# yu45020/Text_Segmentation_Image_Inpainting

Measured on AMD Instinct MI355X. Metric: imgs/sec fwd+bwd on 512x512 partial-conv inpaint, higher is better.
Workload: dtype f32 (storage, accumulation, stencils, BatchNorm; matrix products = 6-term exact bf16 split on the bf16 MFMA, fp32-class error); 1 GPU; ImageFill 512x512 partial-conv inpainting train step (fwd+bwd, train-mode BN, L1 loss, grad all-reduce, fused SGD), 32 imgs/GPU, random line/ellipse hole masks; global_batch=32, parallelism=dp1, gemm_products=6, activation_storage=f32

## Files before the change

### include/tsii_hip.h

```cpp
#ifndef TSII_HIP_H
#define TSII_HIP_H

#include <stddef.h>
#include <stdint.h>

#ifdef __cplusplus
extern "C" {
#endif

#define TSII_ABI_VERSION 23

#define TSII_ACT_NONE 0
#define TSII_ACT_RELU 1
#define TSII_ACT_LEAKY 2
#define TSII_ACT_RELU6 3
#define TSII_ACT_SIGMOID 4

int tsii_version(void);
const char* tsii_last_error(void);

int tsii_set_gemm_products(int products);
int tsii_get_gemm_products(void);


int tsii_mask_channel_sum(const float* mask, int n, int h, int w, int c,
                          int64_t sn, int64_t sh, int64_t sw, int64_t sc,
                          float* plane, void* stream);

int tsii_mask_update(const float* p0, float a0, const float* p1, float a1,
                     int n, int h, int w,
                     int kh, int kw, int sh, int sw, int ph, int pw, int dh, int dw,
                     int ho, int wo, float post_scale, int fill_holes,
                     float* denom, float* new_mask, float* inv, void* stream);
// ... 55 lines not shown
                      int n, int h, int wd, int cout, float* y, void* ws, size_t ws_bytes, void* stream);
int tsii_head_cat_bwd_dx(const float* dy, const float* inv, const float* w, int c1, int c2, const float* r0, const float* r1,
                         int n, int h, int wd, int cout, float* dlow, float* dskip, void* ws, size_t ws_bytes, void* stream);
int tsii_head_cat_bwd_dw(const float* dy, const float* inv, const float* keep, const float* low, const float* skip,
                         int c1, int c2, const float* r0, const float* r1, int n, int h, int wd, int cout,
                         float* dwgt, float* dbias, void* ws, size_t ws_bytes, void* stream);
int tsii_head_cat_low_ok(int n, int h, int wd, int c1, int c2, int cout);
int tsii_head_cat_bwd_low_ok(int n, int h, int wd, int c1, int c2, int cout);
int tsii_head_cat_bwd_low(const float* dy, const float* inv, const float* keep, const float* low, const float* skip,
                          int c1, int c2, const float* r0_low, const float* r1, const float* w, int n, int h, int wd, int cout,
                          float* dwgt, float* dbias, float* dlow, void* ws, size_t ws_bytes, void* stream);
int tsii_head_cat_fwd_low_ok(int n, int h, int wd, int c1, int c2, int cout);
int tsii_head_cat_fwd_low(const float* low, const float* skip, int c1, int c2, const float* r0_low, const float* r1,
                          const float* w, const float* bias, const float* denom, const float* keep,
                          int n, int h, int wd, int cout, float* y, void* stream);
int tsii_head_cat_bwd_dw_low(const float* dy, const float* inv, const float* keep, const float* low, const float* skip,
                             int c1, int c2, const float* r0_low, const float* r1, int n, int h, int wd, int cout,
                             float* dwgt, float* dbias, void* ws, size_t ws_bytes, void* stream);

int tsii_stem_s2d(const float* x, const float* mfull, const float* r0, int split, const float* r1,
                  int n, int h, int w, int c, int pad, float* out, void* stream);
int tsii_stem_w_fwd(const float* w, int cout, int cin, int k, float* w2, void* stream);
int tsii_stem_w_bwd(const float* dw2, int cout, int cin, int k, float* dw, void* stream);

size_t tsii_bn_ws_bytes(int64_t m, int c);
int tsii_bn_stats(const float* y, int64_t m, int c, float* mean, float* var,
                  float* running_mean, float* running_var, float momentum,
                  void* ws, size_t ws_bytes, void* stream);
int tsii_bn_act_fwd(const float* y, int64_t m, int c, const float* mean, const float* var,
                    const float* gamma, const float* beta, float eps, int act, float slope,
                    const float* residual, float* out, void* stream);
int tsii_bn_act_bwd(const float* dout, const float* y, int64_t m, int c,
                    const float* mean, const float* var, const float* gamma, const float* beta,
                    float eps, int act, float slope, int training,
                    float* dy, float* dgamma, float* dbeta, void* ws, size_t ws_bytes, void* stream);

int64_t tsii_pw_stat_rows(int64_t m);
int tsii_pw_fwd_bn(const float* x, int64_t m, int k, const float* w, int n, const float* bias,
                   const float* r0, int split, const float* r1, const float* denom, const float* keep,
                   const float* in_scale, const float* in_shift, int in_act, float in_slope,
                   float* stat_part, float* y, void* ws, size_t ws_bytes, void* stream);
int tsii_pw_bwd_dw_bn(const float* dy, const float* x, int64_t m, int n, int k, const float* inv, const float* keep,
                      const float* r0, int split, const float* r1,
                      const float* in_scale, const float* in_shift, int in_act, float in_slope,
                      float* dw, float* dbias, void* ws, size_t ws_bytes, void* stream);
int64_t tsii_dw_stat_rows(int n, int ho, int wo, int c, int kh, int kw, int sh, int sw, int dh, int dw);
// ... 281 lines not shown
```

### text_segmentation_image_inpainting_amd/BaseModels.py

```python
from contextlib import contextmanager

from typing import NamedTuple, Optional

import torch
from torch import nn

from . import ops


class BaseModule(nn.Module):

    def __init__(self):
        super().__init__()
        self.act_fn = None

    def initialize_weights(self):
        for mod in self.modules():
            weight = getattr(mod, "weight", None)
            if weight is None or not weight.requires_grad:
                continue
            if isinstance(mod, nn.Conv2d):
                nn.init.kaiming_normal_(weight, mode="fan_out", nonlinearity="leaky_relu")
                if mod.bias is not None:
                    nn.init.zeros_(mod.bias)
# ... 249 lines not shown
    return to_nchw(h)


class DSConvBlock(BaseModule):

    def __init__(self, in_channels, out_channels, kernel_size, stride=1, padding=0,
                 dilation=1, bias=True, BN=False, activation_dep=None, activation_point=None):
        super().__init__()
        self.depth_wise_conv = nn.Sequential(
            *Conv_block(in_channels, in_channels, kernel_size, stride, padding,
                        dilation, in_channels, bias, BN=BN, activation=activation_dep))
        self.point_wise_conv = nn.Sequential(
            *Conv_block(in_channels, out_channels, kernel_size=1, stride=1, padding=0,
                        dilation=1, bias=bias, BN=BN, activation=activation_point))

    def forward(self, x):
        return run_chain(list(self.depth_wise_conv) + list(self.point_wise_conv), x)


def run_nhwc(layer, x, mp):
    if hasattr(layer, "forward_nhwc"):
        return layer.forward_nhwc(x, mp)
    if isinstance(layer, nn.Sequential):
        from .partial_convolution import PartialActivatedBN, PartialConv, PartialConv1x1, run_block
        if len(layer) == 2 and isinstance(layer[0], (PartialConv, PartialConv1x1)) and isinstance(layer[1], PartialActivatedBN):
            return run_block(layer, x, mp)
        for m in layer:
            x, mp = run_nhwc(m, x, mp)
        return x, mp
    raise NotImplementedError(f"{type(layer).__name__} is not part of the partial-convolution path")
```

### text_segmentation_image_inpainting_amd/_lib.py

```python
import ctypes
import os

import torch

_HERE = os.path.dirname(os.path.abspath(__file__))
LIB_PATH = os.environ.get("TSII_LIBRARY") or os.path.join(_HERE, "libtsii_hip.so")
ABI_VERSION = 23

_p, _i, _l, _f, _z = ctypes.c_void_p, ctypes.c_int, ctypes.c_int64, ctypes.c_float, ctypes.c_size_t
_GEOM = [_i] * 8

SIGNATURES = {
    "tsii_version": (_i, []),
    "tsii_last_error": (ctypes.c_char_p, []),
    "tsii_set_gemm_products": (_i, [_i]),
    "tsii_get_gemm_products": (_i, []),
    "tsii_mask_channel_sum": (_i, [_p, _i, _i, _i, _i, _l, _l, _l, _l, _p, _p]),
    "tsii_mask_update": (_i, [_p, _f, _p, _f, _i, _i, _i] + _GEOM + [_i, _i, _f, _i, _p, _p, _p, _p]),
    "tsii_plane_upsample2x": (_i, [_p, _i, _i, _i, _p, _p]),
    "tsii_mul_mask": (_i, [_p, _p, _l, _p, _p]),
    "tsii_pw_ws_bytes": (_z, [_i, _i]),
    "tsii_pw_fwd": (_i, [_p, _l, _i, _p, _i, _p, _p, _i, _p, _p, _p, _p, _p, _z, _p]),
    "tsii_pw_bwd_dx": (_i, [_p, _l, _i, _p, _i, _p, _p, _i, _p, _p, _p, _p]),
    "tsii_pw_bwd_dw_ws_bytes": (_z, [_l, _i, _i]),
    "tsii_pw_bwd_dw": (_i, [_p, _p, _l, _i, _i, _p, _p, _p, _i, _p, _p, _p, _p, _z, _p]),
    "tsii_pw_bwd_dxdw_ok": (_i, [_l, _i, _i, _l]),
    "tsii_pw_bwd_dxdw_tiles_per_block": (_i, [_l, _i, _i]),
    "tsii_pw_bwd_dxdw_ws_bytes": (_z, [_l, _i, _i]),
    "tsii_pw_bwd_dxdw": (_i, [_p, _p, _l, _i, _p, _i, _p, _p, _p, _i, _p, _p, _p, _p, _p, _z, _p]),
    "tsii_dw_fwd": (_i, [_p, _p, _p, _p, _p, _p, _i, _i, _i, _i] + _GEOM + [_i, _i, _p, _p, _p]),
    "tsii_dw_bwd_dx": (_i, [_p, _p, _p, _p, _i, _i, _i, _i] + _GEOM + [_i, _i, _p, _p, _p]),
    "tsii_dw_bwd_dw_ws_bytes": (_z, [_i, _i, _i, _i, _i, _i]),
    "tsii_dw_bwd_dw": (_i, [_p, _p, _p, _p, _p, _i, _i, _i, _i] + _GEOM + [_i, _i, _p, _p, _p, _z, _p]),
    "tsii_dense_ws_bytes": (_z, [_i, _i, _i, _i]),
    "tsii_dense_fwd": (_i, [_p, _p, _p, _i, _p, _p, _p, _p, _p, _i, _i, _i, _i, _i] + _GEOM + [_i, _i, _p, _p, _z, _p]),
    "tsii_dense_bwd_dx": (_i, [_p, _p, _p, _p, _p, _i, _p, _i, _i, _i, _i, _i] + _GEOM + [_i, _i, _p, _p, _z, _p]),
    "tsii_head_cat_ok": (_i, [_i, _i, _i, _i, _i, _i]),
    "tsii_head_cat_fwd": (_i, [_p, _p, _i, _i, _p, _p, _p, _p, _p, _p, _i, _i, _i, _i, _p, _p, _z, _p]),
    "tsii_head_cat_bwd_dx": (_i, [_p, _p, _p, _i, _i, _p, _p, _i, _i, _i, _i, _p, _p, _p, _z, _p]),
    "tsii_head_cat_bwd_dw": (_i, [_p, _p, _p, _p, _p, _i, _i, _p, _p, _i, _i, _i, _i, _p, _p, _p, _z, _p]),
    "tsii_head_cat_low_ok": (_i, [_i, _i, _i, _i, _i, _i]),
    "tsii_head_cat_fwd_low_ok": (_i, [_i, _i, _i, _i, _i, _i]),
    "tsii_head_cat_bwd_low_ok": (_i, [_i, _i, _i, _i, _i, _i]),
    "tsii_head_cat_bwd_low": (_i, [_p, _p, _p, _p, _p, _i, _i, _p, _p, _p, _i, _i, _i, _i, _p, _p, _p, _p, _z, _p]),
    "tsii_head_cat_fwd_low": (_i, [_p, _p, _i, _i, _p, _p, _p, _p, _p, _p, _i, _i, _i, _i, _p, _p]),
    "tsii_head_cat_bwd_dw_low": (_i, [_p, _p, _p, _p, _p, _i, _i, _p, _p, _i, _i, _i, _i, _p, _p, _p, _z, _p]),
    "tsii_dense_bwd_dw_ws_bytes": (_z, [_i, _i, _i, _i, _i, _i, _i]),
    "tsii_dense_bwd_dw": (_i, [_p, _p, _p, _p, _p, _p, _i, _p, _i, _i, _i, _i, _i] + _GEOM + [_i, _i, _p, _p, _p, _z, _p]),
    "tsii_stem_s2d": (_i, [_p, _p, _p, _i, _p, _i, _i, _i, _i, _i, _p, _p]),
    "tsii_stem_w_fwd": (_i, [_p, _i, _i, _i, _p, _p]),
    "tsii_stem_w_bwd": (_i, [_p, _i, _i, _i, _p, _p]),
    "tsii_bn_ws_bytes": (_z, [_l, _i]),
    "tsii_bn_stats": (_i, [_p, _l, _i, _p, _p, _p, _p, _f, _p, _z, _p]),
    "tsii_bn_act_fwd": (_i, [_p, _l, _i, _p, _p, _p, _p, _f, _i, _f, _p, _p, _p]),
    "tsii_bn_act_bwd": (_i, [_p, _p, _l, _i, _p, _p, _p, _p, _f, _i, _f, _i, _p, _p, _p, _p, _z, _p]),
    "tsii_pw_fwd_up": (_i, [_p, _l, _i, _p, _i, _p, _p, _i, _p, _p, _p, _p, _i, _i, _p, _p, _p, _z, _p]),
    "tsii_pool2x2_scaled": (_i, [_p, _p, _i, _i, _i, _i, _p, _p]),
    "tsii_pw_stat_rows": (_l, [_l]),
    "tsii_pw_fwd_bn": (_i, [_p, _l, _i, _p, _i, _p, _p, _i, _p, _p, _p, _p, _p, _i, _f, _p, _p, _p, _z, _p]),
    "tsii_pw_bwd_dw_bn": (_i, [_p, _p, _l, _i, _i, _p, _p, _p, _i, _p, _p, _p, _i, _f, _p, _p, _p, _z, _p]),
    "tsii_dw_stat_rows": (_l, [_i, _i, _i, _i, _i, _i, _i, _i, _i, _i]),
    "tsii_dw_bwd_stat_rows": (_l, [_i, _i, _i, _i, _i, _i, _i, _i, _i, _i, _i, _i]),
    "tsii_dw_fwd_bn": (_i, [_p, _p, _p, _p, _p, _p, _i, _i, _i, _i] + _GEOM + [_i, _i, _p, _p, _i, _f, _p, _p, _p, _p]),
    "tsii_dw_bwd_dw_bn": (_i, [_p, _p, _p, _p, _p, _i, _i, _i, _i] + _GEOM + [_i, _i, _p, _p, _i, _f, _p, _p, _p, _z, _p]),
    "tsii_dense_stat_rows": (_l, [_i, _i, _i, _i, _i, _i] + _GEOM + [_i, _i]),
    "tsii_dense_fwd_bn": (_i, [_p, _p, _p, _i, _p, _p, _p, _p, _p, _i, _i, _i, _i, _i] + _GEOM + [_i, _i, _p, _p, _p, _z, _p]),
    "tsii_bn_finalize_ws_bytes": (_z, [_l, _i]),
    "tsii_bn_finalize": (_i, [_p, _l, _i, _l, _p, _p, _p, _p, _f, _p, _p, _f, _p, _p, _p, _z, _p]),
    "tsii_dw_bwd_dx_bn": (_i, [_p, _p, _p, _p, _i, _i, _i, _i] + _GEOM + [_i, _i, _p, _p, _p, _p, _p, _f, _i, _f, _p, _p, _p, _p]),
    "tsii_dw_bwd_dxdw_ws_bytes": (_z, [_i, _i, _i, _i] + _GEOM),
    "tsii_dw_bwd_dxdw_bn": (_i, [_p, _p, _p, _p, _i, _i, _i, _i] + _GEOM + [_i, _i, _p, _p, _p, _p, _p, _f, _i, _f, _p, _p, _p, _p, _p, _z, _p]),
    "tsii_dw_bwd_dxdw_fold_ok": (_i, [_i, _i, _i, _i] + _GEOM),
    "tsii_dw_bwd_dxdw_bn2": (_i, [_p, _p, _p, _i, _f, _p, _p, _p, _i, _i, _i, _i] + _GEOM + [_i, _i, _p, _p, _p, _p, _p, _f, _i, _f, _p, _p, _p, _p, _p, _z, _p]),
    "tsii_bn_bwd_reduce_ws_bytes": (_z, [_l, _i]),
# ... 228 lines not shown
```

### text_segmentation_image_inpainting_amd/build_ext.py

```python
import hashlib
import json
import os
import re
import shutil
import subprocess
import sys
from concurrent.futures import ThreadPoolExecutor

HERE = os.path.dirname(os.path.abspath(__file__))
CSRC = os.path.join(HERE, "csrc")
OBJ = os.path.join(CSRC, "_obj")
LIB = os.path.join(HERE, "libtsii_hip.so")
ARCH = "gfx950"
FLAGS = ["-O3", "-std=c++17", "-fPIC", "--offload-arch=" + ARCH, "-Wall", "-Wno-unused-function"]
RESOURCE_REMARKS = ["-Rpass-analysis=kernel-resource-usage"]
NO_PACKED_F32 = ["-Xclang", "-target-feature", "-Xclang", "-packed-fp32-ops"]
MFMA_SOURCES = ("gemm.hip", "gemm_split.hip", "gemm_pc.hip", "head_mfma.hip", "bf16_gemm.hip", "gemm_dxdw.hip")


def flags_for(src):
    return FLAGS + (NO_PACKED_F32 if os.path.basename(src) in MFMA_SOURCES else [])


def _hipcc():
    for cand in (os.environ.get("HIPCC"), shutil.which("hipcc"), "/opt/rocm/bin/hipcc"):
        if cand and os.path.exists(cand):
            return cand
    raise RuntimeError("hipcc not found (need ROCm to build libtsii_hip.so)")


_REMARK = re.compile(r"remark: +([A-Za-z ]+?)(?: \[[^\]]*\])?: +(\S+)")
_REMARK_CONT = re.compile(r"^\s+\d+ \| |^\s+\| +\^")


def parse_resource_remarks(lines):
    keys = {"VGPRs": "vgprs", "AGPRs": "agprs", "ScratchSize": "scratch", "Occupancy": "occupancy", "LDS Size": "lds", "TotalSGPRs": "sgprs",
            "VGPRs Spill": "vgpr_spill", "SGPRs Spill": "sgpr_spill"}
    out, cur = {}, None
    for ln in lines:
        m = _REMARK.search(ln)
# ... 90 lines not shown
```

### text_segmentation_image_inpainting_amd/ops.py

```python
from typing import NamedTuple, Optional

import torch

from . import _lib
from ._lib import call, ptr

ACT_NONE, ACT_RELU, ACT_LEAKY, ACT_RELU6, ACT_SIGMOID = 0, 1, 2, 3, 4

FUSE_BN_BWD = True
FUSE_BN_BWD_PW = True
FUSE_DW_DXDW = True
FUSE_PW_DXDW = True
PW_DXDW_MIN_M = -1
FUSE_DW_BN2_FOLD = True
BF16_UNFUSE_K6C_ON_LARGE = False
FUSE_POOL_BN_BWD = True
USE_HEAD_MFMA = True
FUSE_HEAD_DLOW = True
USE_STEM_S2D = True


class Geom(NamedTuple):
    kh: int
    kw: int
    sh: int
    sw: int
    ph: int
    pw: int
    dh: int
    dw: int

    def out_hw(self, h, w):
        ho = (h + 2 * self.ph - self.dh * (self.kh - 1) - 1) // self.sh + 1
        wo = (w + 2 * self.pw - self.dw * (self.kw - 1) - 1) // self.sw + 1
        return ho, wo


def _pair(v):
    return (v, v) if isinstance(v, int) else tuple(v)


def make_geom(kernel_size, stride=1, padding=0, dilation=1) -> Geom:
# ... 512 lines not shown
        g = ctx.g
        gy = gy.contiguous()
        n, h, wd, cin = x.shape
        cout = w.shape[0]
        ho, wo = g.out_hw(h, wd)
        L, st = _lib.lib(), _lib.stream()
        dx = dw = db = None
        if ctx.needs_input_grad[0]:
            dx = torch.empty_like(x)
            nbytes = L.tsii_dense_ws_bytes(cin, cout, g.kh, g.kw)
            ws = _ws(nbytes, x)
            call("tsii_dense_bwd_dx", ptr(gy), ptr(inv), ptr(w), ptr(mfull), ptr(r0), ctx.split, ptr(r1),
                 n, h, wd, cin, cout, *g, ho, wo, ptr(dx), ptr(ws), nbytes, st)
        if ctx.needs_input_grad[1] or (ctx.has_bias and ctx.needs_input_grad[2]):
            dw = torch.empty_like(w)
            db = torch.empty(cout, dtype=torch.float32, device=x.device) if ctx.has_bias else None
            nbytes = L.tsii_dense_bwd_dw_ws_bytes(n, ho, wo, cin, cout, g.kh, g.kw)
            ws = _ws(nbytes, x)
            call("tsii_dense_bwd_dw", ptr(gy), ptr(inv), ptr(keep), ptr(x), ptr(mfull), ptr(r0), ctx.split, ptr(r1),
                 n, h, wd, cin, cout, *g, ho, wo, ptr(dw), ptr(db), ptr(ws), nbytes, st)
        return dx, dw, db, None, None, None, None, None, None, None, None, None


class _StemS2D(torch.autograd.Function):

    @staticmethod
    def forward(ctx, x, w, bias, mfull, r0, r1, denom, keep, inv, split, g, want_stats):
        _lib.check_device(x)
        x, w = x.contiguous(), w.contiguous()
        n, h, wd, cin = x.shape
        cout, k, pad = w.shape[0], g.kh, g.ph
        ka, c4 = (k + 1) // 2, 4 * cin
        h2, w2 = (h + 2 * pad) // 2, (wd + 2 * pad) // 2
        ho, wo = g.out_hw(h, wd)
        st, L = _lib.stream(), _lib.lib()
        x2 = torch.empty((n, h2, w2, c4), dtype=torch.float32, device=x.device)
        call("tsii_stem_s2d", ptr(x), ptr(mfull), ptr(r0), int(split), ptr(r1), n, h, wd, cin, pad, ptr(x2), st)
        wk = torch.empty((cout, c4, ka, ka), dtype=torch.float32, device=x.device)
        call("tsii_stem_w_fwd", ptr(w), cout, cin, k, ptr(wk), st)
        g2 = Geom(ka, ka, 1, 1, 0, 0, 1, 1)
        assert g2.out_hw(h2, w2) == (ho, wo)
        y = torch.empty((n, ho, wo, cout), dtype=torch.float32, device=x.device)
        nbytes = L.tsii_dense_ws_bytes(c4, cout, ka, ka)
        ws = _ws(nbytes, x)
        rows = int(L.tsii_dense_stat_rows(0, n, h2, w2, c4, cout, *g2, ho, wo)) if want_stats else 0
        part = None
        if rows > 0:
            part = torch.empty((rows, 4, cout), dtype=torch.float32, device=x.device)
            call("tsii_dense_fwd_bn", ptr(x2), None, None, 0, None, ptr(wk), ptr(bias), ptr(denom), ptr(keep),
                 n, h2, w2, c4, cout, *g2, ho, wo, ptr(part), ptr(y), ptr(ws), nbytes, st)
        else:
            call("tsii_dense_fwd", ptr(x2), None, None, 0, None, ptr(wk), ptr(bias), ptr(denom), ptr(keep),
                 n, h2, w2, c4, cout, *g2, ho, wo, ptr(y), ptr(ws), nbytes, st)
        ctx.save_for_backward(x2, inv, keep)
        ctx.cfg = (tuple(w.shape), g2, (n, h2, w2, c4, ho, wo), bias is not None)
        ctx.set_materialize_grads(False)
        if part is not None:
            ctx.mark_non_differentiable(part)
            return y, part
        return y

    @staticmethod
    def backward(ctx, gy, *_):
        if gy is None:
            return (None,) * 12
        x2, inv, keep = ctx.saved_tensors
        wshape, g2, (n, h2, w2, c4, ho, wo), has_bias = ctx.cfg
        cout, cin, k = wshape[0], wshape[1], wshape[2]
        gy = gy.contiguous()
        L, st = _lib.lib(), _lib.stream()
        dw = db = None
        if ctx.needs_input_grad[1] or (has_bias and ctx.needs_input_grad[2]):
            ka = g2.kh
            dwk = torch.empty((cout, c4, ka, ka), dtype=torch.float32, device=gy.device)
            db = torch.empty(cout, dtype=torch.float32, device=gy.device) if has_bias else None
            nbytes = L.tsii_dense_bwd_dw_ws_bytes(n, ho, wo, c4, cout, ka, ka)
            ws = _ws(nbytes, gy)
            call("tsii_dense_bwd_dw", ptr(gy), ptr(inv), ptr(keep), ptr(x2), None, None, 0, None,
                 n, h2, w2, c4, cout, *g2, ho, wo, ptr(dwk), ptr(db), ptr(ws), nbytes, st)
            dw = torch.empty(wshape, dtype=torch.float32, device=gy.device)
            call("tsii_stem_w_bwd", ptr(dwk), cout, cin, k, ptr(dw), st)
        return (None, dw, db) + (None,) * 9


class _DenseH(torch.autograd.Function):

    @staticmethod
    def forward(ctx, x, w, bias, g, want_stats):
        _lib.check_device(x, bf16_ok=True)
        x, w = x.contiguous(), w.contiguous()
        n, h, wd, cin = x.shape
        cout = w.shape[0]
        assert w.shape[1] == cin, "dense conv needs groups == 1"
        ho, wo = g.out_hw(h, wd)
        L = _lib.lib()
        y = torch.empty((n, ho, wo, cout), dtype=BF16, device=x.device)
        part = torch.empty((int(L.tsii_bf16_stat_rows(n * ho * wo)), 4, cout), dtype=torch.float32, device=x.device) if want_stats else None
        nbytes = L.tsii_bf16_dense_ws_bytes(cin, cout, g.kh, g.kw)
        ws = _ws(nbytes, x)
        call("tsii_bf16_dense_fwd", ptr(x), ptr(w), ptr(bias), n, h, wd, cin, cout, *g, ho, wo, ptr(part), ptr(y), ptr(ws), nbytes, _lib.stream())
        ctx.save_for_backward(x, w)
        ctx.g, ctx.has_bias = g, bias is not None
        ctx.set_materialize_grads(False)
        if want_stats:
# ... 140 lines not shown
    if cout % 8 != 0:
        if cout != 1 or want_stats:
            raise NotImplementedError(f"bf16 storage: {cout} output channels (multiples of 8, or a 1-channel head without BatchNorm)")
        w8 = torch.cat([w, w.new_zeros((7,) + tuple(w.shape[1:]))], 0)
        b8 = None if bias is None else torch.cat([bias, bias.new_zeros(7)], 0)
        return _ChannelToF32.apply(_DenseH.apply(x, w8, b8, g, False), 0)
    return _DenseH.apply(x, w, bias, g, want_stats)


def _stem_form(x, w, g: Geom):
    cin, cout = x.shape[-1], w.shape[0]
    return (USE_STEM_S2D and not x.requires_grad and g.kh == g.kw and g.kh % 2 == 1 and g.kh >= 3 and g.sh == g.sw == 2 and
            g.ph == g.pw == (g.kh - 1) // 2 and g.dh == g.dw == 1 and cin <= 4 and cout % 4 == 0 and cout >= 16 and
            (x.shape[1] + 2 * g.ph) % 2 == 0 and (x.shape[2] + 2 * g.pw) % 2 == 0)


def _bf16_stem_form(x, w, g: Geom):
    cin, cout = x.shape[-1], w.shape[0]
    return (not x.requires_grad and g.kh == g.kw and g.kh % 2 == 1 and g.kh >= 3 and g.sh == g.sw == 2 and
            g.ph == g.pw == (g.kh - 1) // 2 and g.dh == g.dw == 1 and cin <= 4 and cout % 8 == 0 and cout >= 16 and
            (x.shape[1] + 2 * g.ph) % 2 == 0 and (x.shape[2] + 2 * g.pw) % 2 == 0)


def pconv_dense(x, w, bias, mfull, r0, split, r1, denom, keep, inv, g: Geom, want_stats=False):
    data_layer = (_ACT_STORAGE == BF16 and x.dtype == torch.float32 and x.shape[-1] <= 4 and
                  mfull is None and r0 is None and denom is None)
    if data_layer and not _bf16_stem_form(x, w, g):
        raise NotImplementedError("bf16 activation storage: the data layer cannot enter it (needs an odd-k stride-2 'same' stem over "
                                  f"<= 4 channels with Cout % 8 == 0, even padded size and no input gradient; got k={g.kh}x{g.kw} "
                                  f"stride={g.sh} cin={x.shape[-1]} cout={w.shape[0]} requires_grad={x.requires_grad})")
    if _h(x) or data_layer:
        _no_masks("dense convolution", mfull, r0, r1, denom, keep)
        out = _dense_bf16(x, w, bias, g, want_stats)
        return (out, None) if (want_stats and not isinstance(out, tuple)) else out
    if _stem_form(x, w, g):
        out = _StemS2D.apply(x, w, bias, mfull, r0, r1, denom, keep, inv, split, g, want_stats)
    else:
        out = _Dense.apply(x, w, bias, mfull, r0, r1, denom, keep, inv, split, g, want_stats)
    if want_stats and not isinstance(out, tuple):
        return out, None
    return out


class _BNAct(torch.autograd.Function):
    @staticmethod
    def forward(ctx, y, gamma, beta, running_mean, running_var, residual, training, momentum, eps, act, slope, part=None):
        _lib.check_device(y)
        y = y.contiguous()
        c = y.shape[-1]
        m = y.numel() // c
        st = _lib.stream()
        if training:
            mean = torch.empty(c, dtype=torch.float32, device=y.device)
            var = torch.empty(c, dtype=torch.float32, device=y.device)
            if part is not None:
                rows = part.shape[0]
                nbytes = _lib.lib().tsii_bn_finalize_ws_bytes(rows, c)
# ... 803 lines not shown
```

### text_segmentation_image_inpainting_amd/partial_convolution.py

```python
import torch
from torch import nn

from . import ops
from .BaseModels import BaseModule, act_code, bn_state, to_nchw, to_nhwc
from .masks import MaskParts, as_parts

FUSE_BN = "1"
FUSE_UPCAT = True

inplace_batch_norm = False


def _public_forward(module, args, **kw):
    x, mask = args
    keep_parts = isinstance(mask, MaskParts)
    y, mp = module.forward_nhwc(to_nhwc(x), as_parts(mask), **kw)
    return to_nchw(y), (mp if keep_parts else mp.as_tensor())


class PartialConv(BaseModule):
    def __init__(self, in_channels, out_channels, kernel_size, stride=1,
                 padding=0, dilation=1, groups=1, bias=True, same_holes=False):
        super().__init__()
        self.feature_conv = nn.Conv2d(in_channels, out_channels, kernel_size, stride,
                                      padding, dilation, groups, bias)
        nn.init.kaiming_normal_(self.feature_conv.weight)
        self.same_holes = same_holes
        mask_in = 1 if same_holes else in_channels
        mask_out = 1 if same_holes else out_channels
        mask_groups = 1 if same_holes else groups
        self.mask_conv = nn.Conv2d(mask_in, mask_out, kernel_size, stride,
                                   padding, dilation, mask_groups, bias=False)
        torch.nn.init.constant_(self.mask_conv.weight, 1.0)
        for param in self.mask_conv.parameters():
            param.requires_grad = False

    fill_holes = True

    def _geom(self):
        fc = self.feature_conv
        return ops.make_geom(fc.kernel_size, fc.stride, fc.padding, fc.dilation)

    def forward_nhwc(self, x, mp, want_stats=False):
        fc = self.feature_conv
        w, b = fc.weight, fc.bias
        cin, cout, groups = fc.in_channels, fc.out_channels, fc.groups
        g = self._geom()
        if x.shape[-1] != cin or mp.channels != cin:
            raise RuntimeError(f"PartialConv expects {cin} input channels, got x:{x.shape[-1]} mask:{mp.channels}")
        if self.same_holes:
            p0, a0, p1, a1, post = mp.first_channel_plane(), 1.0, None, 0.0, float(cin)
        elif groups == 1:
            (p0, a0, p1, a1), post = mp.count_operands(), 1.0
        else:
            raise NotImplementedError("grouped PartialConv without same_holes (per-group mask counts, "
                                      "models/partial_convolution.py:63) is not used by any reference "
                                      "network and has no HIP kernel")
        denom, new_mask, inv = ops.mask_update(p0, a0, p1, a1, g, post, self.fill_holes)
        keep = new_mask if self.fill_holes else None
        pointwise = tuple(g) == (1, 1, 1, 1, 0, 0, 1, 1)
        part = None
        real = lambda t: t.materialize() if isinstance(t, ops.LazyBN) else t
        if isinstance(x, ops.VirtualCat):
            if (groups == 1 and mp.fusable and not want_stats and len(mp.parts) == 2 and mp.parts[0].channels == x.low.shape[3]
                    and ops.head_cat_ok(x, cout, g)):
                r0, _, r1 = mp.row_scale()
                y = ops.pconv_head_cat(x, w, b, r0, r1, denom, keep, inv)
                return y, MaskParts.from_plane(new_mask, cout)
            if (groups == 1 and pointwise and mp.fusable and len(mp.parts) == 2 and mp.parts[0].channels == x.low.shape[3]
                    and FUSE_UPCAT and ops.pointwise_up_ok(x, cout)):
                _, cl, r1 = mp.row_scale()
                z = ops.pconv_pointwise(x.low, w[:, :cl], None, x.low_plane, cl, None)
                y = ops.pconv_pointwise(x.skip, w[:, cl:], b, r1, cin - cl, None, denom, keep, inv, want_stats=want_stats, up_add=z)
                if want_stats:
                    y, part = y
                new_mp = MaskParts.from_plane(new_mask, cout)
                return (y, new_mp, part) if want_stats else (y, new_mp)
            x = x.materialize()
        if groups == 1:
            if mp.fusable:
                r0, split, r1 = mp.row_scale()
                if pointwise:
                    y = ops.pconv_pointwise(x, w, b, r0, split, r1, denom, keep, inv, want_stats=want_stats)
                    if want_stats:
                        y, part = y
                else:
                    y = ops.pconv_dense(real(x), w, b, None, r0, split, r1, denom, keep, inv, g, want_stats=want_stats)
                    if want_stats:
                        y, part = y
            else:
                mfull = mp.full_nhwc()
                if pointwise:
                    y = ops.pconv_pointwise(ops.mul_mask(real(x), mfull), w, b, None, 0, None, denom, keep, inv,
                                            want_stats=want_stats)
                    if want_stats:
                        y, part = y
                else:
                    y = ops.pconv_dense(real(x), w, b, mfull, None, 0, None, denom, keep, inv, g, want_stats=want_stats)
                    if want_stats:
                        y, part = y
        elif groups == cin == cout:
            if mp.fusable and len(mp.parts) == 1:
                y = ops.pconv_depthwise(x, w, b, mp.parts[0].plane, denom, keep, inv, g, want_stats=want_stats)
            else:
                y = ops.pconv_depthwise(ops.mul_mask(real(x), mp.full_nhwc()), w, b, None, denom, keep, inv, g,
                                        want_stats=want_stats)
            if want_stats:
                y, part = y
        else:
            raise NotImplementedError(f"PartialConv groups={groups} (neither 1 nor depth-wise) has no HIP kernel")
        new_mp = MaskParts.from_plane(new_mask, cout)
        return (y, new_mp, part) if want_stats else (y, new_mp)

    def forward(self, args):
        return _public_forward(self, args)


class PartialConv1x1(BaseModule):

    def __init__(self, in_channels, out_channels, kernel_size=1, stride=1,
                 padding=0, dilation=1, groups=1, bias=True):
# ... 71 lines not shown
        return ops.activation(x, act, slope), mp

    def forward(self, args):
        return _public_forward(self, args)


class DoubleUpSample(nn.Module):

    def __init__(self, scale_factor, mode="nearest"):
        super().__init__()
        if scale_factor != 2 or mode != "nearest":
            raise NotImplementedError("only the nearest x2 up-sampling the reference networks use has a HIP kernel")
        self.upsample = nn.Upsample(scale_factor=scale_factor, mode=mode)

    def forward_nhwc(self, x, mp):
        if not (mp.fusable and len(mp.parts) == 1 and mp.parts[0].planar):
            up = ops.upsample2x(mp.full_nhwc())
            from .masks import Part
            return ops.upsample2x(x), MaskParts([Part(mp.channels, full=up)])
        return ops.upsample2x(x), mp.upsample2x()

    def forward(self, args):
        return _public_forward(self, args)


def run_block(block, x, mp, allow_lazy=False, residual=None):
    mods = list(block)
    conv_types = (PartialConv, PartialConv1x1)
    if FUSE_BN != "0" and len(mods) == 2 and isinstance(mods[0], conv_types) and isinstance(mods[1], PartialActivatedBN):
        conv, bn = mods
        bn0 = bn.bn_act[0]
        if bn0.training or bn0.running_mean is None:
            y, m, part = conv.forward_nhwc(x, mp, want_stats=True)
        else:
            (y, m), part = conv.forward_nhwc(x, mp), None
        lazy, m = bn.forward_lazy(y, m, part)
        if allow_lazy and residual is None and FUSE_BN == "1" and ops.load_time_act(lazy.act, lazy.slope):
            return lazy, m
        return lazy.materialize(residual), m
    for mod in mods:
        if isinstance(x, ops.LazyBN) and not isinstance(mod, conv_types):
            x = x.materialize()
        x, mp = mod.forward_nhwc(x, mp)
    if isinstance(x, ops.LazyBN):
        x = x.materialize()
    if residual is not None:
# ... 19 lines not shown
```

Baseline: 573.8 imgs/s.

## Add fused stem backward kernel folding LeakyReLU grad into split-bf16 weight gradient

```diff
diff --git a/include/tsii_hip.h b/include/tsii_hip.h
--- a/include/tsii_hip.h
+++ b/include/tsii_hip.h
@@ -8,7 +8,7 @@
 extern "C" {
 #endif
 
-#define TSII_ABI_VERSION 23
+#define TSII_ABI_VERSION 24
 
 #define TSII_ACT_NONE 0
 #define TSII_ACT_RELU 1
@@ -110,6 +110,13 @@
                   int n, int h, int w, int c, int pad, float* out, void* stream);
 int tsii_stem_w_fwd(const float* w, int cout, int cin, int k, float* w2, void* stream);
 int tsii_stem_w_bwd(const float* dw2, int cout, int cin, int k, float* dw, void* stream);
+int tsii_stem_bwd_ok(const float* gy, const float* y, const float* x2, int n, int h2, int w2, int c4, int cout,
+                     int kh, int kw, int stride, int ho, int wo);
+int tsii_stem_bwd_tiles_per_block(int n, int ho, int wo);
+size_t tsii_stem_bwd_ws_bytes(int n, int ho, int wo);
+int tsii_stem_bwd(const float* gy, const float* y, float slope, const float* inv, const float* keep, const float* x2,
+                  int n, int h2, int w2, int c4, int cout, int kh, int kw, int stride, int ho, int wo,
+                  float* dwk, float* db, void* ws, size_t ws_bytes, void* stream);
 
 size_t tsii_bn_ws_bytes(int64_t m, int c);
 int tsii_bn_stats(const float* y, int64_t m, int c, float* mean, float* var,
diff --git a/text_segmentation_image_inpainting_amd/BaseModels.py b/text_segmentation_image_inpainting_amd/BaseModels.py
--- a/text_segmentation_image_inpainting_amd/BaseModels.py
+++ b/text_segmentation_image_inpainting_amd/BaseModels.py
@@ -295,9 +295,11 @@
     if hasattr(layer, "forward_nhwc"):
         return layer.forward_nhwc(x, mp)
     if isinstance(layer, nn.Sequential):
-        from .partial_convolution import PartialActivatedBN, PartialConv, PartialConv1x1, run_block
+        from .partial_convolution import PartialActivatedBN, PartialConv, PartialConv1x1, run_block, stem_act_block
         if len(layer) == 2 and isinstance(layer[0], (PartialConv, PartialConv1x1)) and isinstance(layer[1], PartialActivatedBN):
             return run_block(layer, x, mp)
+        if stem_act_block(layer, x):
+            return layer[0].forward_nhwc(x, mp, act_after=act_code(layer[1].act_fn))
         for m in layer:
             x, mp = run_nhwc(m, x, mp)
         return x, mp
diff --git a/text_segmentation_image_inpainting_amd/_lib.py b/text_segmentation_image_inpainting_amd/_lib.py
--- a/text_segmentation_image_inpainting_amd/_lib.py
+++ b/text_segmentation_image_inpainting_amd/_lib.py
@@ -5,7 +5,7 @@
 
 _HERE = os.path.dirname(os.path.abspath(__file__))
 LIB_PATH = os.environ.get("TSII_LIBRARY") or os.path.join(_HERE, "libtsii_hip.so")
-ABI_VERSION = 23
+ABI_VERSION = 24
 
 _p, _i, _l, _f, _z = ctypes.c_void_p, ctypes.c_int, ctypes.c_int64, ctypes.c_float, ctypes.c_size_t
 _GEOM = [_i] * 8
@@ -50,6 +50,10 @@
     "tsii_stem_s2d": (_i, [_p, _p, _p, _i, _p, _i, _i, _i, _i, _i, _p, _p]),
     "tsii_stem_w_fwd": (_i, [_p, _i, _i, _i, _p, _p]),
     "tsii_stem_w_bwd": (_i, [_p, _i, _i, _i, _p, _p]),
+    "tsii_stem_bwd_ok": (_i, [_p, _p, _p] + [_i] * 10),
+    "tsii_stem_bwd_tiles_per_block": (_i, [_i, _i, _i]),
+    "tsii_stem_bwd_ws_bytes": (_z, [_i, _i, _i]),
+    "tsii_stem_bwd": (_i, [_p, _p, _f, _p, _p, _p] + [_i] * 10 + [_p, _p, _p, _z, _p]),
     "tsii_bn_ws_bytes": (_z, [_l, _i]),
     "tsii_bn_stats": (_i, [_p, _l, _i, _p, _p, _p, _p, _f, _p, _z, _p]),
     "tsii_bn_act_fwd": (_i, [_p, _l, _i, _p, _p, _p, _p, _f, _i, _f, _p, _p, _p]),
diff --git a/text_segmentation_image_inpainting_amd/build_ext.py b/text_segmentation_image_inpainting_amd/build_ext.py
--- a/text_segmentation_image_inpainting_amd/build_ext.py
+++ b/text_segmentation_image_inpainting_amd/build_ext.py
@@ -15,7 +15,7 @@
 FLAGS = ["-O3", "-std=c++17", "-fPIC", "--offload-arch=" + ARCH, "-Wall", "-Wno-unused-function"]
 RESOURCE_REMARKS = ["-Rpass-analysis=kernel-resource-usage"]
 NO_PACKED_F32 = ["-Xclang", "-target-feature", "-Xclang", "-packed-fp32-ops"]
-MFMA_SOURCES = ("gemm.hip", "gemm_split.hip", "gemm_pc.hip", "head_mfma.hip", "bf16_gemm.hip", "gemm_dxdw.hip")
+MFMA_SOURCES = ("gemm.hip", "gemm_split.hip", "gemm_pc.hip", "head_mfma.hip", "bf16_gemm.hip", "gemm_dxdw.hip", "stem_bwd.hip")
 
 
 def flags_for(src):
diff --git a/text_segmentation_image_inpainting_amd/csrc/stem_bwd.hip b/text_segmentation_image_inpainting_amd/csrc/stem_bwd.hip
--- /dev/null
+++ b/text_segmentation_image_inpainting_amd/csrc/stem_bwd.hip
@@ -0,0 +1,286 @@
+#include "bf16_common.h"
+#include "gemm_tiles.h"
+#include "split_bf16.h"
+
+namespace tsii {
+
+static constexpr int SB_ROWS = 64;
+static constexpr int SB_SUB = 3 * SB_ROWS * 64;
+static constexpr int SB_C4 = 12, SB_KA = 4, SB_COUT = 64;
+static constexpr int SB_K = SB_C4 * SB_KA * SB_KA;
+static constexpr int SB_WIN_FLOATS = (SB_ROWS + SB_KA - 1) * SB_C4;
+static constexpr int SB_WIN_CHUNKS = (SB_WIN_FLOATS + 7) / 8;
+static constexpr int SB_WIN_ROW = SB_WIN_CHUNKS * 16;
+static constexpr int SB_WIN_PLANE = SB_KA * SB_WIN_ROW;
+static constexpr int SB_ROW_STEP = SB_C4 * 2;
+static constexpr int SB_SLAB = SB_K * SB_COUT + SB_COUT;
+
+#if defined(TSII_HIP_EMU)
+template <class... T> static inline void sb_lds_wait(T&...) {}
+#else
+__device__ __forceinline__ void sb_lds_wait(hu32x2& a, hu32x2& b, hu32x2& c, hu32x2& d, hu32x2& e, hu32x2& f) {
+    asm volatile("s_waitcnt lgkmcnt(0)" : "+v"(a), "+v"(b), "+v"(c), "+v"(d), "+v"(e), "+v"(f) : : "memory");
+}
+#endif
+
+__device__ __forceinline__ void sb_operand(hu32x2 (&lo)[3], hu32x2 (&hi)[3], bf16x8 (&o)[3]) {
+    sb_lds_wait(lo[0], hi[0], lo[1], hi[1], lo[2], hi[2]);
+#pragma unroll
+    for (int p = 0; p < 3; ++p) {
+        const u32x4 v = {lo[p][0], lo[p][1], hi[p][0], hi[p][1]};
+        o[p] = __builtin_bit_cast(bf16x8, v);
+    }
+}
+
+template <int KS>
+__device__ __forceinline__ void sb_step(const unsigned char* __restrict__ Gb, int tro0, int tro1, const unsigned char* (&Wa)[3], f32x16 (&acc)[3]) {
+    hu32x2 bl[3], bh[3];
+    bf16x8 b[3];
+    lds_read8_tr<KS * 1024>(bl[0], Gb + tro0);
+    lds_read8_tr<KS * 1024>(bh[0], Gb + tro1);
+    lds_read8_tr<KS * 1024 + SB_ROWS * 64>(bl[1], Gb + tro0);
+    lds_read8_tr<KS * 1024 + SB_ROWS * 64>(bh[1], Gb + tro1);
+    lds_read8_tr<KS * 1024 + 2 * SB_ROWS * 64>(bl[2], Gb + tro0);
+    lds_read8_tr<KS * 1024 + 2 * SB_ROWS * 64>(bh[2], Gb + tro1);
+    sb_operand(bl, bh, b);
+#pragma unroll
+    for (int s = 0; s < 3; ++s) {
+        constexpr int O = KS * 16 * SB_ROW_STEP;
+        hu32x2 al[3], ah[3];
+        bf16x8 a[3];
+        lds_read8_tr<O>(al[0], Wa[s]);
+        lds_read8_tr<O + 4 * SB_ROW_STEP>(ah[0], Wa[s]);
+        lds_read8_tr<O + SB_WIN_PLANE>(al[1], Wa[s]);
+        lds_read8_tr<O + SB_WIN_PLANE + 4 * SB_ROW_STEP>(ah[1], Wa[s]);
+        lds_read8_tr<O + 2 * SB_WIN_PLANE>(al[2], Wa[s]);
+        lds_read8_tr<O + 2 * SB_WIN_PLANE + 4 * SB_ROW_STEP>(ah[2], Wa[s]);
+        sb_operand(al, ah, a);
+#pragma unroll
+        for (int pq = 0; pq < 6; ++pq)
+            acc[s] = __builtin_amdgcn_mfma_f32_32x32x16_bf16(a[SplitTerm<6>::pa(pq)], b[SplitTerm<6>::pb(pq)], acc[s], 0, 0, 0);
+    }
+}
+
+__device__ __forceinline__ void sb_unpack(const float4 (&r)[2], float (&v)[8]) {
+    v[0] = r[0].x; v[1] = r[0].y; v[2] = r[0].z; v[3] = r[0].w; v[4] = r[1].x; v[5] = r[1].y; v[6] = r[1].z; v[7] = r[1].w;
+}
+
+template <bool ACT>
+__global__ __launch_bounds__(256, 2) void stem_bwd_kernel(const float* __restrict__ gy, const float* __restrict__ y, float slope,
+                                                          const float* __restrict__ inv, const float* __restrict__ keep,
+                                                          const float* __restrict__ x2, int ho, int wo, float* __restrict__ part,
+                                                          int ntiles, int tiles_per_block) {
+    __shared__ __attribute__((aligned(16))) unsigned char smem[2 * SB_SUB + 3 * SB_WIN_PLANE];
+    unsigned char* Gs = smem;
+    unsigned char* Wn = smem + 2 * SB_SUB;
+
+    const int tid = threadIdx.x, lane = tid & 63, wave = tid >> 6;
+    const int li = lane & 31, hi = lane >> 5;
+    const int wr = wave >> 1, wu = wave & 1;
+    const int tile_beg = (int)blockIdx.x * tiles_per_block;
+    const int tile_end = tile_beg + tiles_per_block < ntiles ? tile_beg + tiles_per_block : ntiles;
+    const int h2 = ho + SB_KA - 1, w2 = wo + SB_KA - 1, tiles_per_row = wo >> 6;
+
+    f32x16 acc[3];
+#pragma unroll
+    for (int s = 0; s < 3; ++s)
+#pragma unroll
+        for (int r = 0; r < 16; ++r) acc[s][r] = 0.f;
+    float dbacc[2][8];
+#pragma unroll
+    for (int h = 0; h < 2; ++h)
+#pragma unroll
+        for (int e = 0; e < 8; ++e) dbacc[h][e] = 0.f;
+
+    unsigned woff[2][2];
+    int wlds[2];
+    bool wvalid[2];
+#pragma unroll
+    for (int i = 0; i < 2; ++i) {
+        const int f = tid + 256 * i;
+        wvalid[i] = f < SB_KA * SB_WIN_CHUNKS;
+        const int fc = wvalid[i] ? f : SB_KA * SB_WIN_CHUNKS - 1;
+        const int ay = fc / SB_WIN_CHUNKS, ch = fc - ay * SB_WIN_CHUNKS;
+        woff[i][0] = (unsigned)((ay * w2 * SB_C4 + 8 * ch) * 4);
+        woff[i][1] = woff[i][0] + (8 * ch + 4 < SB_WIN_FLOATS ? 16u : 0u);
+        wlds[i] = ay * SB_WIN_ROW + ch * 16;
+    }
+
+    float4 rg[2][1][2], ry[2][1][2], rw[2][2];
+    float finv = 1.f, fkeep = 1.f;
+    auto prefetch = [&](int tile) {
+        const int64_t row0 = (int64_t)tile * SB_ROWS;
+        const int orow = tile / tiles_per_row, ox0 = (tile - orow * tiles_per_row) * SB_ROWS;
+        const int img = orow / ho, oy = orow - img * ho;
+        const char* xb = reinterpret_cast<const char*>(x2 + (((int64_t)img * h2 + oy) * w2 + ox0) * SB_C4);
+#pragma unroll
+        for (int i = 0; i < 2; ++i) {
+            rw[i][0] = *reinterpret_cast<const float4*>(xb + woff[i][0]);
+            rw[i][1] = *reinterpret_cast<const float4*>(xb + woff[i][1]);
+        }
+#pragma unroll
+        for (int h = 0; h < 2; ++h) {
+            split_load<SB_ROWS>(gy + row0 * SB_COUT, SB_COUT, 0, SB_ROWS, 32 * h, SB_COUT, rg[h]);
+            if constexpr (ACT) split_load<SB_ROWS>(y + row0 * SB_COUT, SB_COUT, 0, SB_ROWS, 32 * h, SB_COUT, ry[h]);
+        }
+        const int64_t row = row0 + (tid >> 2);
+        finv = inv != nullptr ? inv[row] : 1.f;
+        fkeep = keep != nullptr ? keep[row] : 1.f;
+    };
+
+    const int q = lane & 15, g1 = (lane >> 4) & 1;
+    int tro[2];
+#pragma unroll
+    for (int j = 0; j < 2; ++j) {
+        const int row = 8 * hi + (q >> 2) + 4 * j, chunk = 2 * g1 + ((q & 3) >> 1);
+        tro[j] = row * 64 + ((chunk ^ ((2 * hi + j) & 3)) << 4) + (q & 1) * 8;
+    }
+    const unsigned char* Gb = Gs + wu * SB_SUB;
+    const unsigned char* Wa[3];
+#pragma unroll
+    for (int s = 0; s < 3; ++s) {
+        const int b = 2 * (2 * s + wr) + g1, ay = b / 3, jb = b - 3 * ay;
+        Wa[s] = Wn + ay * SB_WIN_ROW + (8 * hi + (q >> 2)) * SB_ROW_STEP + (16 * jb + 4 * (q & 3)) * 2;
+    }
+
+    if (tile_beg < tile_end) prefetch(tile_beg);
+    for (int tile = tile_beg; tile < tile_end; ++tile) {
+        __syncthreads();
+#pragma unroll
+        for (int i = 0; i < 2; ++i) {
+            if (wvalid[i]) {
+                float v[8];
+                sb_unpack(rw[i], v);
+                u32x4 pl[3];
+                split8<3>(v, pl);
+#pragma unroll
+                for (int p = 0; p < 3; ++p) *reinterpret_cast<u32x4*>(Wn + p * SB_WIN_PLANE + wlds[i]) = pl[p];
+            }
+        }
+#pragma unroll
+        for (int h = 0; h < 2; ++h) {
+            float v[8];
+            sb_unpack(rg[h][0], v);
+            if constexpr (ACT) {
+                float a[8];
+                sb_unpack(ry[h][0], a);
+#pragma unroll
+                for (int e = 0; e < 8; ++e) v[e] = v[e] * (a[e] > 0.f ? 1.f : slope);
+                rg[h][0][0] = make_float4(v[0], v[1], v[2], v[3]);
+                rg[h][0][1] = make_float4(v[4], v[5], v[6], v[7]);
+            }
+#pragma unroll
+            for (int e = 0; e < 8; ++e) dbacc[h][e] += v[e] * fkeep;
+            const float s0[1] = {finv}, s1[1] = {finv};
+            const float4 z = make_float4(0.f, 0.f, 0.f, 0.f);
+            const float4 none[2] = {z, z};
+            split_store<SB_ROWS, 3, true, false>(Gs + h * SB_SUB, rg[h], 32 * h, 0x7fffffff, s0, s1, none, none, 1.f, 0.f, SB_ROWS, SB_COUT);
+        }
+        __syncthreads();
+        prefetch(tile + 1 < tile_end ? tile + 1 : tile);
+        __builtin_amdgcn_s_setprio(2);
+        sb_step<0>(Gb, tro[0], tro[1], Wa, acc);
+        sb_step<1>(Gb, tro[0], tro[1], Wa, acc);
+        sb_step<2>(Gb, tro[0], tro[1], Wa, acc);
+        sb_step<3>(Gb, tro[0], tro[1], Wa, acc);
+        __builtin_amdgcn_s_setprio(0);
+    }
+
+    float* pz = part + (int64_t)blockIdx.x * SB_SLAB;
+#pragma unroll
+    for (int s = 0; s < 3; ++s)
+#pragma unroll
+        for (int r = 0; r < 16; ++r) {
+            const int k = 32 * (2 * s + wr) + (r & 3) + 8 * (r >> 2) + 4 * hi;
+            pz[k * SB_COUT + 32 * wu + li] = acc[s][r];
+        }
+    __syncthreads();
+    float* Ds = reinterpret_cast<float*>(Gs);
+#pragma unroll
+    for (int h = 0; h < 2; ++h)
+#pragma unroll
+        for (int e = 0; e < 8; ++e) Ds[(tid >> 2) * SB_COUT + 32 * h + 8 * (tid & 3) + e] = dbacc[h][e];
+    __syncthreads();
+    if (tid < SB_COUT) {
+        float t = 0.f;
+        for (int r = 0; r < SB_ROWS; ++r) t += Ds[r * SB_COUT + tid];
+        pz[SB_K * SB_COUT + tid] = t;
+    }
+}
+
+__global__ void stem_bwd_finish_kernel(const float* __restrict__ red, float* __restrict__ dwk, float* __restrict__ db) {
+    const int o = (int)(blockIdx.x * blockDim.x + threadIdx.x);
+    if (o < SB_K * SB_COUT) {
+        const int co = o / SB_K, rem = o - co * SB_K;
+        const int c = rem >> 4, ay = (rem >> 2) & 3, ax = rem & 3;
+        dwk[o] = red[(48 * ay + 12 * ax + c) * SB_COUT + co];
+    } else if (o < SB_SLAB && db != nullptr) {
+        db[o - SB_K * SB_COUT] = red[o];
+    }
+}
+
+static bool sb_geom_ok(int n, int h2, int w2, int c4, int cout, int kh, int kw, int stride, int ho, int wo) {
+    if (n <= 0 || ho <= 0 || wo <= 0 || c4 != SB_C4 || cout != SB_COUT || kh != SB_KA || kw != SB_KA || stride != 1) return false;
+    if (wo % SB_ROWS != 0 || wo > (1 << 20) || h2 != ho + SB_KA - 1 || w2 != wo + SB_KA - 1) return false;
+    return (int64_t)n * ho * (wo / SB_ROWS) < (1ll << 31);
+}
+
+static void sb_plan(int n, int ho, int wo, int* nblocks, int* tiles_per_block) {
+    const int64_t ntiles = (int64_t)n * ho * (wo / SB_ROWS);
+    int64_t want = (int64_t)device_cus() * 2;
+    if (want > ntiles) want = ntiles;
+    const int64_t tpb = cdiv64(ntiles, want);
+    *tiles_per_block = (int)tpb;
+    *nblocks = (int)cdiv64(ntiles, tpb);
+}
+
+}
+
+using namespace tsii;
+
+extern "C" int tsii_stem_bwd_ok(const float* gy, const float* y, const float* x2, int n, int h2, int w2, int c4, int cout,
+                                int kh, int kw, int stride, int ho, int wo) {
+    if (gemm_products() != 6) return 0;
+    if (!sb_geom_ok(n, h2, w2, c4, cout, kh, kw, stride, ho, wo)) return 0;
+    return (gy != nullptr && x2 != nullptr && aligned16(gy) && aligned16(x2) && aligned16(y)) ? 1 : 0;
+}
+
+extern "C" int tsii_stem_bwd_tiles_per_block(int n, int ho, int wo) {
+    if (!sb_geom_ok(n, ho + SB_KA - 1, wo + SB_KA - 1, SB_C4, SB_COUT, SB_KA, SB_KA, 1, ho, wo)) return 0;
+    int nb = 0, tpb = 0;
+    sb_plan(n, ho, wo, &nb, &tpb);
+    return tpb;
+}
+
+extern "C" size_t tsii_stem_bwd_ws_bytes(int n, int ho, int wo) {
+    if (!sb_geom_ok(n, ho + SB_KA - 1, wo + SB_KA - 1, SB_C4, SB_COUT, SB_KA, SB_KA, 1, ho, wo)) return 0;
+    int nb = 0, tpb = 0;
+    sb_plan(n, ho, wo, &nb, &tpb);
+    return ((size_t)nb + 1) * SB_SLAB * sizeof(float);
+}
+
+extern "C" int tsii_stem_bwd(const float* gy, const float* y, float slope, const float* inv, const float* keep, const float* x2,
+                             int n, int h2, int w2, int c4, int cout, int kh, int kw, int stride, int ho, int wo,
+                             float* dwk, float* db, void* ws, size_t ws_bytes, void* stream) {
+    TSII_REQUIRE(gy && x2 && dwk && ws, "stem_bwd: null pointer");
+    TSII_REQUIRE(gemm_products() == 6, "stem_bwd: the 6-product split-bf16 arithmetic only (tsii_set_gemm_products)");
+    TSII_REQUIRE(sb_geom_ok(n, h2, w2, c4, cout, kh, kw, stride, ho, wo),
+                 "stem_bwd: n=%d x2 %dx%dx%d cout=%d taps %dx%d stride %d out %dx%d is not eligible (tsii_stem_bwd_ok)", n, h2, w2, c4, cout, kh,
+                 kw, stride, ho, wo);
+    TSII_REQUIRE(aligned16(gy) && aligned16(y) && aligned16(x2) && aligned16(ws), "stem_bwd: 16-byte aligned operands are required");
+    TSII_REQUIRE(ws_bytes >= tsii_stem_bwd_ws_bytes(n, ho, wo), "stem_bwd: workspace too small");
+    hipStream_t st = (hipStream_t)stream;
+    int nb = 0, tpb = 0;
+    sb_plan(n, ho, wo, &nb, &tpb);
+    const int ntiles = (int)((int64_t)n * ho * (wo / SB_ROWS));
+    float* part = (float*)ws;
+    float* red = part + (size_t)nb * SB_SLAB;
+    if (y != nullptr) hipLaunchKernelGGL((stem_bwd_kernel<true>), dim3(nb), dim3(256), 0, st, gy, y, slope, inv, keep, x2, ho, wo, part, ntiles, tpb);
+    else hipLaunchKernelGGL((stem_bwd_kernel<false>), dim3(nb), dim3(256), 0, st, gy, y, slope, inv, keep, x2, ho, wo, part, ntiles, tpb);
+    int rc = check_launch("stem_bwd");
+    if (rc) return rc;
+    rc = launch_reduce_rows(part, nb, SB_SLAB, red, st);
+    if (rc) return rc;
+    hipLaunchKernelGGL(stem_bwd_finish_kernel, dim3(cdiv(SB_SLAB, 256)), dim3(256), 0, st, red, dwk, db);
+    return check_launch("stem_bwd_finish");
+}
diff --git a/text_segmentation_image_inpainting_amd/ops.py b/text_segmentation_image_inpainting_amd/ops.py
--- a/text_segmentation_image_inpainting_amd/ops.py
+++ b/text_segmentation_image_inpainting_amd/ops.py
@@ -18,6 +18,7 @@
 USE_HEAD_MFMA = True
 FUSE_HEAD_DLOW = True
 USE_STEM_S2D = True
+FUSE_STEM_BWD = True
 
 
 class Geom(NamedTuple):
@@ -576,38 +577,72 @@
         return dx, dw, db, None, None, None, None, None, None, None, None, None
 
 
+def _stem_forward(ctx, x, w, bias, mfull, r0, r1, denom, keep, inv, split, g, want_stats):
+    _lib.check_device(x)
+    x, w = x.contiguous(), w.contiguous()
+    n, h, wd, cin = x.shape
+    cout, k, pad = w.shape[0], g.kh, g.ph
+    ka, c4 = (k + 1) // 2, 4 * cin
+    h2, w2 = (h + 2 * pad) // 2, (wd + 2 * pad) // 2
+    ho, wo = g.out_hw(h, wd)
+    st, L = _lib.stream(), _lib.lib()
+    x2 = torch.empty((n, h2, w2, c4), dtype=torch.float32, device=x.device)
+    call("tsii_stem_s2d", ptr(x), ptr(mfull), ptr(r0), int(split), ptr(r1), n, h, wd, cin, pad, ptr(x2), st)
+    wk = torch.empty((cout, c4, ka, ka), dtype=torch.float32, device=x.device)
+    call("tsii_stem_w_fwd", ptr(w), cout, cin, k, ptr(wk), st)
+    g2 = Geom(ka, ka, 1, 1, 0, 0, 1, 1)
+    assert g2.out_hw(h2, w2) == (ho, wo)
+    y = torch.empty((n, ho, wo, cout), dtype=torch.float32, device=x.device)
+    nbytes = L.tsii_dense_ws_bytes(c4, cout, ka, ka)
+    ws = _ws(nbytes, x)
+    rows = int(L.tsii_dense_stat_rows(0, n, h2, w2, c4, cout, *g2, ho, wo)) if want_stats else 0
+    part = None
+    if rows > 0:
+        part = torch.empty((rows, 4, cout), dtype=torch.float32, device=x.device)
+        call("tsii_dense_fwd_bn", ptr(x2), None, None, 0, None, ptr(wk), ptr(bias), ptr(denom), ptr(keep),
+             n, h2, w2, c4, cout, *g2, ho, wo, ptr(part), ptr(y), ptr(ws), nbytes, st)
+    else:
+        call("tsii_dense_fwd", ptr(x2), None, None, 0, None, ptr(wk), ptr(bias), ptr(denom), ptr(keep),
+             n, h2, w2, c4, cout, *g2, ho, wo, ptr(y), ptr(ws), nbytes, st)
+    ctx.cfg = (tuple(w.shape), g2, (n, h2, w2, c4, ho, wo), bias is not None)
+    return y, part, x2
+
+
+def _stem_backward(ctx, x2, inv, keep, gy, y=None, slope=0.0):
+    wshape, g2, (n, h2, w2, c4, ho, wo), has_bias = ctx.cfg
+    cout, cin, k = wshape[0], wshape[1], wshape[2]
+    if not (ctx.needs_input_grad[1] or (has_bias and ctx.needs_input_grad[2])):
+        return None, None
+    gy = gy.contiguous()
+    L, st = _lib.lib(), _lib.stream()
+    ka = g2.kh
+    dwk = torch.empty((cout, c4, ka, ka), dtype=torch.float32, device=gy.device)
+    db = torch.empty(cout, dtype=torch.float32, device=gy.device) if has_bias else None
+    if FUSE_STEM_BWD and L.tsii_stem_bwd_ok(ptr(gy), ptr(y), ptr(x2), n, h2, w2, c4, cout, ka, ka, 1, ho, wo):
+        nbytes = L.tsii_stem_bwd_ws_bytes(n, ho, wo)
+        ws = _ws(nbytes, gy)
+        call("tsii_stem_bwd", ptr(gy), ptr(y), float(slope), ptr(inv), ptr(keep), ptr(x2), n, h2, w2, c4, cout, ka, ka, 1, ho, wo,
+             ptr(dwk), ptr(db), ptr(ws), nbytes, st)
+    else:
+        if y is not None:
+            dy = torch.empty_like(gy)
+            call("tsii_act_bwd", ptr(gy), ptr(y), gy.numel(), ACT_LEAKY, float(slope), ptr(dy), st)
+            gy = dy
+        nbytes = L.tsii_dense_bwd_dw_ws_bytes(n, ho, wo, c4, cout, ka, ka)
+        ws = _ws(nbytes, gy)
+        call("tsii_dense_bwd_dw", ptr(gy), ptr(inv), ptr(keep), ptr(x2), None, None, 0, None,
+             n, h2, w2, c4, cout, *g2, ho, wo, ptr(dwk), ptr(db), ptr(ws), nbytes, st)
+    dw = torch.empty(wshape, dtype=torch.float32, device=gy.device)
+    call("tsii_stem_w_bwd", ptr(dwk), cout, cin, k, ptr(dw), st)
+    return dw, db
+
+
 class _StemS2D(torch.autograd.Function):
 
     @staticmethod
     def forward(ctx, x, w, bias, mfull, r0, r1, denom, keep, inv, split, g, want_stats):
-        _lib.check_device(x)
-        x, w = x.contiguous(), w.contiguous()
-        n, h, wd, cin = x.shape
-        cout, k, pad = w.shape[0], g.kh, g.ph
-        ka, c4 = (k + 1) // 2, 4 * cin
-        h2, w2 = (h + 2 * pad) // 2, (wd + 2 * pad) // 2
-        ho, wo = g.out_hw(h, wd)
-        st, L = _lib.stream(), _lib.lib()
-        x2 = torch.empty((n, h2, w2, c4), dtype=torch.float32, device=x.device)
-        call("tsii_stem_s2d", ptr(x), ptr(mfull), ptr(r0), int(split), ptr(r1), n, h, wd, cin, pad, ptr(x2), st)
-        wk = torch.empty((cout, c4, ka, ka), dtype=torch.float32, device=x.device)
-        call("tsii_stem_w_fwd", ptr(w), cout, cin, k, ptr(wk), st)
-        g2 = Geom(ka, ka, 1, 1, 0, 0, 1, 1)
-        assert g2.out_hw(h2, w2) == (ho, wo)
-        y = torch.empty((n, ho, wo, cout), dtype=torch.float32, device=x.device)
-        nbytes = L.tsii_dense_ws_bytes(c4, cout, ka, ka)
-        ws = _ws(nbytes, x)
-        rows = int(L.tsii_dense_stat_rows(0, n, h2, w2, c4, cout, *g2, ho, wo)) if want_stats else 0
-        part = None
-        if rows > 0:
-            part = torch.empty((rows, 4, cout), dtype=torch.float32, device=x.device)
-            call("tsii_dense_fwd_bn", ptr(x2), None, None, 0, None, ptr(wk), ptr(bias), ptr(denom), ptr(keep),
-                 n, h2, w2, c4, cout, *g2, ho, wo, ptr(part), ptr(y), ptr(ws), nbytes, st)
-        else:
-            call("tsii_dense_fwd", ptr(x2), None, None, 0, None, ptr(wk), ptr(bias), ptr(denom), ptr(keep),
-                 n, h2, w2, c4, cout, *g2, ho, wo, ptr(y), ptr(ws), nbytes, st)
+        y, part, x2 = _stem_forward(ctx, x, w, bias, mfull, r0, r1, denom, keep, inv, split, g, want_stats)
         ctx.save_for_backward(x2, inv, keep)
-        ctx.cfg = (tuple(w.shape), g2, (n, h2, w2, c4, ho, wo), bias is not None)
         ctx.set_materialize_grads(False)
         if part is not None:
             ctx.mark_non_differentiable(part)
@@ -619,21 +654,28 @@
         if gy is None:
             return (None,) * 12
         x2, inv, keep = ctx.saved_tensors
-        wshape, g2, (n, h2, w2, c4, ho, wo), has_bias = ctx.cfg
-        cout, cin, k = wshape[0], wshape[1], wshape[2]
-        gy = gy.contiguous()
-        L, st = _lib.lib(), _lib.stream()
-        dw = db = None
-        if ctx.needs_input_grad[1] or (has_bias and ctx.needs_input_grad[2]):
-            ka = g2.kh
-            dwk = torch.empty((cout, c4, ka, ka), dtype=torch.float32, device=gy.device)
-            db = torch.empty(cout, dtype=torch.float32, device=gy.device) if has_bias else None
-            nbytes = L.tsii_dense_bwd_dw_ws_bytes(n, ho, wo, c4, cout, ka, ka)
-            ws = _ws(nbytes, gy)
-            call("tsii_dense_bwd_dw", ptr(gy), ptr(inv), ptr(keep), ptr(x2), None, None, 0, None,
-                 n, h2, w2, c4, cout, *g2, ho, wo, ptr(dwk), ptr(db), ptr(ws), nbytes, st)
-            dw = torch.empty(wshape, dtype=torch.float32, device=gy.device)
-            call("tsii_stem_w_bwd", ptr(dwk), cout, cin, k, ptr(dw), st)
+        dw, db = _stem_backward(ctx, x2, inv, keep, gy)
+        return (None, dw, db) + (None,) * 9
+
+
+class _StemS2DAct(torch.autograd.Function):
+
+    @staticmethod
+    def forward(ctx, x, w, bias, mfull, r0, r1, denom, keep, inv, split, g, slope):
+        y, _, x2 = _stem_forward(ctx, x, w, bias, mfull, r0, r1, denom, keep, inv, split, g, False)
+        out = torch.empty_like(y)
+        call("tsii_act_fwd", ptr(y), y.numel(), ACT_LEAKY, float(slope), ptr(out), _lib.stream())
+        ctx.save_for_backward(x2, inv, keep, y)
+        ctx.slope = float(slope)
+        ctx.set_materialize_grads(False)
+        return out
+
+    @staticmethod
+    def backward(ctx, gout):
+        if gout is None:
+            return (None,) * 12
+        x2, inv, keep, y = ctx.saved_tensors
+        dw, db = _stem_backward(ctx, x2, inv, keep, gout, y, ctx.slope)
         return (None, dw, db) + (None,) * 9
 
 
@@ -820,7 +862,14 @@
             (x.shape[1] + 2 * g.ph) % 2 == 0 and (x.shape[2] + 2 * g.pw) % 2 == 0)
 
 
-def pconv_dense(x, w, bias, mfull, r0, split, r1, denom, keep, inv, g: Geom, want_stats=False):
+def _stem_bwd_form(x, w, g: Geom):
+    if not (FUSE_STEM_BWD and _ACT_STORAGE != BF16 and isinstance(x, torch.Tensor) and x.dtype == torch.float32 and _stem_form(x, w, g)):
+        return False
+    wo = g.out_hw(x.shape[1], x.shape[2])[1]
+    return (x.shape[-1] == 3 and g.kh == 7 and w.shape[0] == 64 and wo % 64 == 0 and int(_lib.lib().tsii_get_gemm_products()) == 6)
+
+
+def pconv_dense(x, w, bias, mfull, r0, split, r1, denom, keep, inv, g: Geom, want_stats=False, act_after=None):
     data_layer = (_ACT_STORAGE == BF16 and x.dtype == torch.float32 and x.shape[-1] <= 4 and
                   mfull is None and r0 is None and denom is None)
     if data_layer and not _bf16_stem_form(x, w, g):
@@ -831,6 +880,9 @@
         _no_masks("dense convolution", mfull, r0, r1, denom, keep)
         out = _dense_bf16(x, w, bias, g, want_stats)
         return (out, None) if (want_stats and not isinstance(out, tuple)) else out
+    if act_after is not None:
+        assert act_after[0] == ACT_LEAKY and not want_stats and _stem_bwd_form(x, w, g)
+        return _StemS2DAct.apply(x, w, bias, mfull, r0, r1, denom, keep, inv, split, g, float(act_after[1]))
     if _stem_form(x, w, g):
         out = _StemS2D.apply(x, w, bias, mfull, r0, r1, denom, keep, inv, split, g, want_stats)
     else:
diff --git a/text_segmentation_image_inpainting_amd/partial_convolution.py b/text_segmentation_image_inpainting_amd/partial_convolution.py
--- a/text_segmentation_image_inpainting_amd/partial_convolution.py
+++ b/text_segmentation_image_inpainting_amd/partial_convolution.py
@@ -41,7 +41,7 @@
         fc = self.feature_conv
         return ops.make_geom(fc.kernel_size, fc.stride, fc.padding, fc.dilation)
 
-    def forward_nhwc(self, x, mp, want_stats=False):
+    def forward_nhwc(self, x, mp, want_stats=False, act_after=None):
         fc = self.feature_conv
         w, b = fc.weight, fc.bias
         cin, cout, groups = fc.in_channels, fc.out_channels, fc.groups
@@ -85,7 +85,7 @@
                     if want_stats:
                         y, part = y
                 else:
-                    y = ops.pconv_dense(real(x), w, b, None, r0, split, r1, denom, keep, inv, g, want_stats=want_stats)
+                    y = ops.pconv_dense(real(x), w, b, None, r0, split, r1, denom, keep, inv, g, want_stats=want_stats, act_after=act_after)
                     if want_stats:
                         y, part = y
             else:
@@ -96,7 +96,7 @@
                     if want_stats:
                         y, part = y
                 else:
-                    y = ops.pconv_dense(real(x), w, b, mfull, None, 0, None, denom, keep, inv, g, want_stats=want_stats)
+                    y = ops.pconv_dense(real(x), w, b, mfull, None, 0, None, denom, keep, inv, g, want_stats=want_stats, act_after=act_after)
                     if want_stats:
                         y, part = y
         elif groups == cin == cout:
@@ -214,6 +214,14 @@
 
     def forward(self, args):
         return _public_forward(self, args)
+
+
+def stem_act_block(layer, x):
+    if not (ops.FUSE_STEM_BWD and len(layer) == 2 and isinstance(layer[0], PartialConv) and isinstance(layer[1], PartialActivation)
+            and isinstance(x, torch.Tensor) and isinstance(layer[1].act_fn, nn.LeakyReLU)):
+        return False
+    fc = layer[0].feature_conv
+    return fc.groups == 1 and ops._stem_bwd_form(x, fc.weight, layer[0]._geom())
 
 
 def run_block(block, x, mp, allow_lazy=False, residual=None):
```

New measurement: 583.0 imgs/s (median of 6 runs). +1.6%, better.
